# ZhengyiLuo/PULSE

Hardware: NVIDIA H100
Metric: env-steps/sec at 16384 humanoid envs, 1/2/4/8 H100; obs-kernel HBM GB/s (higher is better)
Workload: dtype bf16 GEMM operands, fp32 accumulate / master weights / observations

## Files before the change

### pulse_b200/csrc/gemm_kernel.inc

```
#if PULSE_GEMM_GROUPED
#define PULSE_GEMM_FIRST(member) grp.p[0].member
#define PULSE_GEMM_W wl
#define PULSE_GEMM_SELECT(w)                                                                                         \
  int pi = 0;                                                                                                        \
  while (pi + 1 < grp.count && (w) >= grp.p[pi].item_end) ++pi;                                                      \
  const GemmProblem& P = grp.p[pi];                                                                                  \
  const int wl = (w) - (pi == 0 ? 0 : grp.p[pi - 1].item_end);                                                       \
  const CUtensorMap& map_a = P.map_a;                                                                                \
  const CUtensorMap& map_b = P.map_b;                                                                                \
  const CUtensorMap& map_c = P.map_c;                                                                                \
  const int use_tma_red = P.use_tma_red;                                                                             \
  const pulse_gemm_epilogue_t& ep = P.ep;                                                                            \
  const int M = P.M, N = P.N, K = P.K, kb_per_split = P.kb_per_split;                                                \
  const int tiles_n = (N + BN - 1) / BN, tiles_m = (M + BM - 1) / BM;                                                \
  const int tiles = tiles_m * tiles_n;                                                                               \
  const int num_kb_total = (K + BK - 1) / BK;                                                                        \
  (void)map_a; (void)map_b; (void)map_c; (void)use_tma_red; (void)ep; (void)M; (void)N; (void)tiles_n; (void)kb_per_split; (void)num_kb_total;
#else
#define PULSE_GEMM_FIRST(member) member
#define PULSE_GEMM_W w
#define PULSE_GEMM_SELECT(w)
#endif

#if PULSE_GEMM_GROUPED
template <bool A_MN, bool B_MN, int MODE>
__global__ void __launch_bounds__(kThreads, 1) gemm_bf16_grouped_kernel(const __grid_constant__ GemmGroup grp) {
#else
template <bool A_MN, bool B_MN, int MODE>
__global__ void __launch_bounds__(kThreads, 1) gemm_bf16_kernel(const __grid_constant__ CUtensorMap map_a,
                                                                const __grid_constant__ CUtensorMap map_b,
                                                                const __grid_constant__ CUtensorMap map_c,
                                                                const pulse_gemm_epilogue_t ep, int M, int N, int K,
                                                                int kb_per_split, int splits, int use_tma_red) {
#endif
  constexpr bool kFwd = MODE == kModeGeneric || MODE == kModeFwd;
  constexpr bool kDgrad = MODE == kModeGeneric || MODE == kModeDgrad || MODE == kModeDgradVec;
  constexpr bool kGateVec = MODE == kModeGeneric || MODE == kModeDgradVec;
  constexpr bool kAccum = MODE == kModeGeneric || MODE == kModeWgrad;
  constexpr bool kBf16Out = MODE != kModeWgrad;
  extern __shared__ unsigned char gsm_raw[];
  GemmSmem& sm = *reinterpret_cast<GemmSmem*>((reinterpret_cast<uintptr_t>(gsm_raw) + 1023) & ~static_cast<uintptr_t>(1023));
  const int warp = threadIdx.x >> 5, lane = threadIdx.x & 31;
  const int work0 = static_cast<int>(blockIdx.x);
  const int work_stride = static_cast<int>(gridDim.x);
#if PULSE_GEMM_GROUPED
  const int total = grp.total_items;
#else
  const int tiles_n = (N + BN - 1) / BN, tiles_m = (M + BM - 1) / BM;
  const int tiles = tiles_m * tiles_n;
  const int total = tiles * splits;
  const int num_kb_total = (K + BK - 1) / BK;
#endif
  if (threadIdx.x == 0) PULSE_TRACE(0);

  if (threadIdx.x == 0) {
#pragma unroll
    for (int s = 0; s < kStages; ++s) {
      g_mbar_init(&sm.full[s], 1);
      g_mbar_init(&sm.empty[s], kConsumerWarps);
    }
    asm volatile("fence.mbarrier_init.release.cluster;\n" ::: "memory");
    asm volatile("prefetch.tensormap [%0];\n" ::"l"(&PULSE_GEMM_FIRST(map_a)) : "memory");
    asm volatile("prefetch.tensormap [%0];\n" ::"l"(&PULSE_GEMM_FIRST(map_b)) : "memory");
  }
  __syncthreads();
  if (threadIdx.x == 0) PULSE_TRACE(1);
  asm volatile("griddepcontrol.launch_dependents;\n" ::: "memory");

  if (warp < 4) {
    if (warp == 0 && lane == 0) {
      asm volatile("griddepcontrol.wait;\n" ::: "memory");
      PULSE_TRACE(2);
// ... 9 lines not shown
          g_mbar_wait(&sm.empty[s], ((it / kStages) & 1) ^ 1);
          g_mbar_expect_tx(&sm.full[s], kStageBytesA + kStageBytesB);
          const int kk = (kb0 + kb) * BK;
          if (A_MN) {
            tma_load_2d(sm.a[s], &map_a, m0, kk, &sm.full[s]);
            tma_load_2d(sm.a[s] + 8192, &map_a, m0 + 64, kk, &sm.full[s]);
          } else {
            tma_load_2d(sm.a[s], &map_a, kk, m0, &sm.full[s]);
          }
          if (B_MN) {
            tma_load_2d(sm.b[s], &map_b, n0, kk, &sm.full[s]);
            tma_load_2d(sm.b[s] + 8192, &map_b, n0 + 64, kk, &sm.full[s]);
          } else {
            tma_load_2d(sm.b[s], &map_b, kk, n0, &sm.full[s]);
          }
        }
      }
    }
  } else {
    const int wg = (warp >> 2) - 1;
    const int ew = warp - 4;
    const int quarter = wg * 2 + (warp & 1);
    const int chalf = (warp >> 1) & 1;
    float* red_stage = sm.red[ew];
    float* acc_s = sm.acc[wg];
    asm volatile("griddepcontrol.wait;\n" ::: "memory");
    int it = 0, lw = 0;
    for (int w = work0; w < total; w += work_stride, ++lw) {
      PULSE_GEMM_SELECT(w)
      const int split = PULSE_GEMM_W / tiles, t = PULSE_GEMM_W - split * tiles;
      const int m0 = (t / tiles_n) * BM, n0 = (t % tiles_n) * BN;
      const int kb0 = split * kb_per_split;
      const int num_kb = min(kb_per_split, num_kb_total - kb0);
      const int row = m0 + quarter * 32 + lane;
      const bool row_ok = row < M;
      const bool gate_fast = (MODE == kModeGeneric || MODE == kModeDgrad) && ep.gate != nullptr && ep.gate_mask == nullptr && ep.gate_mode == PULSE_ACT_RELU && (ep.ldg & 7) == 0 && n0 + chalf * kCols + kCols <= N;
      unsigned gmask[kChunks] = {};
      const bool gate_bits = kDgrad && ep.gate_mask != nullptr;
      if (gate_bits && row_ok) {
#pragma unroll
        for (int cc = 0; cc < kChunks; ++cc) {
          const int col = n0 + (chalf * kChunks + cc) * 32;
          if (col < N) gmask[cc] = __ldg(ep.gate_mask + static_cast<long long>(col >> 5) * ep.ld_gmask + row);
        }
      }
      if (gate_fast && row_ok) {
        const uint4* g = reinterpret_cast<const uint4*>(reinterpret_cast<const __nv_bfloat16*>(ep.gate) + static_cast<long long>(row) * ep.ldg +
                                                        n0 + chalf * kCols);
        uint4 u[kChunks * 4];
#pragma unroll
        for (int i = 0; i < kChunks * 4; ++i) u[i] = __ldg(g + i);
#pragma unroll
        for (int i = 0; i < kChunks * 4; ++i) {
          const unsigned wds[4] = {u[i].x, u[i].y, u[i].z, u[i].w};
#pragma unroll
          for (int q = 0; q < 4; ++q) {
            const unsigned pos = (((wds[q] & 0x7fff7fffu) + 0x7fff7fffu) & ~wds[q]) & 0x80008000u;
            gmask[i >> 2] |= (pos >> 15) << ((i & 3) * 4 + q);
          }
        }
      }
      const bool gate_vec = kGateVec && ep.gate != nullptr && !gate_fast && !gate_bits && (ep.ldg & 7) == 0;
      uint4 gq[4] = {};
      auto gate_fetch = [&](int cc) {
        const int c0 = n0 + cc * 32;
        if (gate_vec && row_ok && c0 + 32 <= N) {
          const uint4* g = reinterpret_cast<const uint4*>(reinterpret_cast<const __nv_bfloat16*>(ep.gate) + static_cast<long long>(row) * ep.ldg + c0);
#pragma unroll
          for (int q = 0; q < 4; ++q) gq[q] = __ldg(g + q);
        }
      };
      gate_fetch(chalf * kChunks);
      float bias_l[kChunks] = {};
      const bool fwd_fast = MODE == kModeFwd && ep.out != nullptr && (ep.ldo & 7) == 0 && ep.out_f32 == nullptr && ep.out_t == nullptr &&
                            (ep.preact == nullptr || (ep.ldp & 7) == 0) && n0 + chalf * kCols + kCols <= N;
      float* bias_s = sm.bias[ew];
      if (fwd_fast && ep.bias != nullptr) {
        __syncwarp();
#pragma unroll
        for (int cc = 0; cc < kChunks; ++cc) bias_s[cc * 32 + lane] = __ldg(ep.bias + n0 + (chalf * kChunks + cc) * 32 + lane);
        __syncwarp();
      } else if (kFwd && ep.bias != nullptr) {
#pragma unroll
        for (int cc = 0; cc < kChunks; ++cc) {
          const int col = n0 + (chalf * kChunks + cc) * 32 + lane;
          if (col < N) bias_l[cc] = __ldg(ep.bias + col);
        }
      }

      float d[64];
#pragma unroll
      for (int i = 0; i < 64; ++i) d[i] = 0.0f;
      acc_fence(d);
      int prev_s = -1;
      for (int kb = 0; kb < num_kb; ++kb, ++it) {
        const int s = it % kStages;
        g_mbar_wait(&sm.full[s], (it / kStages) & 1);
        if (it == 0 && ew == 0 && lane == 0) PULSE_TRACE(3);
        wgmma_fence();
        const unsigned a_addr = s_u32(sm.a[s]) + static_cast<unsigned>(wg) * 8192u, b_addr = s_u32(sm.b[s]);
#pragma unroll
        for (int k = 0; k < BK / MMA_K; ++k) {
          const unsigned long long da = A_MN ? gmma_desc(a_addr + k * 2048, 8192) : gmma_desc(a_addr + k * 32, 16);
          const unsigned long long db = B_MN ? gmma_desc(b_addr + k * 2048, 8192) : gmma_desc(b_addr + k * 32, 16);
          wgmma_m64n128<A_MN ? 1 : 0, B_MN ? 1 : 0>(d, da, db, (kb | k) != 0 ? 1u : 0u);
        }
        wgmma_commit();
        wgmma_wait<1>();
        if (prev_s >= 0 && lane == 0) g_mbar_arrive(&sm.empty[prev_s]);
        prev_s = s;
      }
      wgmma_wait<0>();
      acc_fence(d);
      if (lane == 0) g_mbar_arrive(&sm.empty[prev_s]);
      if (ew == 0 && lane == 0 && lw < 3) PULSE_TRACE(4 + lw);

      wg_sync(wg);
      {
        const int r0 = (warp & 3) * 16 + (lane >> 2);
#pragma unroll
        for (int j = 0; j < BN / 8; ++j) {
          const int col = 8 * j + 2 * (lane & 3);
#pragma unroll
          for (int h = 0; h < 2; ++h) {
            const int r = r0 + 8 * h;
            const int rb = r & 31;
            float* blk = acc_s + ((r >> 5) * 4 + (col >> 5)) * 1024;
            const int unit = ((col & 31) >> 2) ^ (rb & 7);
            *reinterpret_cast<float2*>(blk + rb * 32 + unit * 4 + (col & 3)) = make_float2(d[4 * j + 2 * h], d[4 * j + 2 * h + 1]);
          }
        }
      }
      if (MODE == kModeWgrad && use_tma_red) asm volatile("fence.proxy.async.shared::cta;\n" ::: "memory");
      wg_sync(wg);
      if (ew == 0 && lane == 0 && lw < 3) PULSE_TRACE(16 + 2 * lw);

      float* outf = ep.out_f32 != nullptr ? ep.out_f32 + static_cast<long long>(ep.accumulate ? 0 : split) * ep.split_stride : nullptr;
      float sq = 0.0f;
#pragma unroll 1
      for (int c = chalf * kChunks; c < chalf * kChunks + kChunks; ++c) {
        const int col0 = n0 + c * 32;
        const bool full = col0 + 32 <= N;
        float* blk = acc_s + ((quarter & 1) * 4 + c) * 1024;
        if (MODE == kModeWgrad && use_tma_red) {
          if (lane == 0) {
            asm volatile("cp.reduce.async.bulk.tensor.2d.global.shared::cta.add.tile.bulk_group [%0, {%2, %3}], [%1];\n" ::"l"(&map_c),
                         "r"(s_u32(blk)), "r"(col0), "r"(m0 + quarter * 32)
                         : "memory");
            asm volatile("cp.async.bulk.commit_group;\n" ::: "memory");
          }
          continue;
        }
        float v[32];
        {
          const float4* b4 = reinterpret_cast<const float4*>(blk) + lane * 8;
#pragma unroll
          for (int u = 0; u < 8; ++u) {
            const float4 x = b4[u ^ (lane & 7)];
            v[4 * u] = x.x; v[4 * u + 1] = x.y; v[4 * u + 2] = x.z; v[4 * u + 3] = x.w;
          }
        }
        if (MODE != kModeWgrad && ep.alpha != 1.0f) {
#pragma unroll
          for (int i = 0; i < 32; ++i) v[i] *= ep.alpha;
        }
        if (fwd_fast) {
          if (ep.bias != nullptr) {
            const float4* b4 = reinterpret_cast<const float4*>(bias_s + (c % kChunks) * 32);
#pragma unroll
            for (int i = 0; i < 32; i += 4) {
              const float4 b = b4[i >> 2];
              v[i] += b.x; v[i + 1] += b.y; v[i + 2] += b.z; v[i + 3] += b.w;
            }
          }
          if (ep.relu_mask != nullptr) {
            unsigned word = 0u;
#pragma unroll
            for (int i = 0; i < 32; ++i) word |= (v[i] > 0.0f ? 1u : 0u) << i;
            if (row_ok) ep.relu_mask[static_cast<long long>(col0 >> 5) * ep.ld_rmask + row] = word;
          }
          uint4* st = reinterpret_cast<uint4*>(red_stage);
          const int sw = (lane >> 1) & 3;
#pragma unroll
          for (int q = 0; q < 4; ++q) {
            const int i = 8 * q;
            __nv_bfloat162 h0 = __floats2bfloat162_rn(v[i], v[i + 1]), h1 = __floats2bfloat162_rn(v[i + 2], v[i + 3]);
            __nv_bfloat162 h2 = __floats2bfloat162_rn(v[i + 4], v[i + 5]), h3 = __floats2bfloat162_rn(v[i + 6], v[i + 7]);
            uint4 u;
            u.x = *reinterpret_cast<unsigned*>(&h0);
            u.y = *reinterpret_cast<unsigned*>(&h1);
            u.z = *reinterpret_cast<unsigned*>(&h2);
            u.w = *reinterpret_cast<unsigned*>(&h3);
            st[lane * 4 + (q ^ sw)] = u;
          }
          __syncwarp();
          const long long coff = col0 + (lane & 3) * 8;
          const __nv_bfloat162 zero2 = __float2bfloat162_rn(0.0f);
#pragma unroll
          for (int it2 = 0; it2 < 4; ++it2) {
            const int rr = it2 * 8 + (lane >> 2);
            uint4 u = st[rr * 4 + ((lane & 3) ^ ((rr >> 1) & 3))];
            __nv_bfloat162* h = reinterpret_cast<__nv_bfloat162*>(&u);
            const long long grow = m0 + quarter * 32 + rr;
            if (grow < M) {
              if (ep.preact != nullptr) *reinterpret_cast<uint4*>(reinterpret_cast<__nv_bfloat16*>(ep.preact) + grow * ep.ldp + coff) = u;
              if (ep.act == PULSE_ACT_RELU) {
#pragma unroll
                for (int q = 0; q < 4; ++q) h[q] = __hmax2(h[q], zero2);
              } else if (ep.act == PULSE_ACT_SILU) {
#pragma unroll
                for (int q = 0; q < 4; ++q) h[q] = silu_bf16x2(h[q]);
              }
              *reinterpret_cast<uint4*>(reinterpret_cast<__nv_bfloat16*>(ep.out) + grow * ep.ldo + coff) = u;
            }
          }
          __syncwarp();
          continue;
        }
        if (kFwd && ep.bias != nullptr) {
          float bl = bias_l[0];
#pragma unroll
          for (int cc = 1; cc < kChunks; ++cc) bl = (c % kChunks) == cc ? bias_l[cc] : bl;
#pragma unroll
          for (int i = 0; i < 32; ++i) v[i] += __shfl_sync(0xffffffffu, bl, i);
        }
        if (kFwd && ep.preact != nullptr) {
          if (full && (ep.ldp & 7) == 0) {
            store_block_bf16(reinterpret_cast<uint4*>(red_stage), v,
                             reinterpret_cast<__nv_bfloat16*>(ep.preact) + static_cast<long long>(m0 + quarter * 32) * ep.ldp + col0, ep.ldp,
                             M - (m0 + quarter * 32), lane);
          } else if (row_ok) {
            __nv_bfloat16* p = reinterpret_cast<__nv_bfloat16*>(ep.preact) + static_cast<long long>(row) * ep.ldp + col0;
#pragma unroll
            for (int i = 0; i < 32; ++i)
              if (col0 + i < N) p[i] = __float2bfloat16(v[i]);
          }
        }
        if (kFwd && ep.relu_mask != nullptr && row_ok) {
          unsigned word = 0u;
#pragma unroll
          for (int i = 0; i < 32; ++i) word |= ((col0 + i < N && v[i] > 0.0f) ? 1u : 0u) << i;
          if (col0 < N) ep.relu_mask[static_cast<long long>(col0 >> 5) * ep.ld_rmask + row] = word;
        }
        if (kFwd && ep.act != PULSE_ACT_NONE) {
#pragma unroll
          for (int i = 0; i < 32; ++i) v[i] = act_apply(v[i], ep.act);
        }
        if (gate_bits) {
          unsigned mk = gmask[0];
#pragma unroll
// ... 64 lines not shown
            }
            __syncwarp();
          }
        } else if (outf != nullptr && row_ok) {
          float* p = outf + static_cast<long long>(row) * ep.ldf + col0;
          if (full && (ep.ldf & 3) == 0 && (reinterpret_cast<uintptr_t>(outf) & 15u) == 0) {
#pragma unroll
            for (int i = 0; i < 32; i += 4) *reinterpret_cast<float4*>(p + i) = make_float4(v[i], v[i + 1], v[i + 2], v[i + 3]);
          } else {
#pragma unroll
            for (int i = 0; i < 32; ++i)
              if (col0 + i < N) p[i] = v[i];
          }
        }
        if (kBf16Out && ep.out != nullptr) {
          if (full && (ep.ldo & 7) == 0) {
            store_block_bf16(reinterpret_cast<uint4*>(red_stage), v,
                             reinterpret_cast<__nv_bfloat16*>(ep.out) + static_cast<long long>(m0 + quarter * 32) * ep.ldo + col0, ep.ldo,
                             M - (m0 + quarter * 32), lane);
          } else if (row_ok) {
            __nv_bfloat16* p = reinterpret_cast<__nv_bfloat16*>(ep.out) + static_cast<long long>(row) * ep.ldo + col0;
#pragma unroll
            for (int i = 0; i < 32; ++i)
              if (col0 + i < N) p[i] = __float2bfloat16(v[i]);
          }
        }
        if (kFwd && ep.out_t != nullptr && row_ok) {
#pragma unroll
          for (int i = 0; i < 32; ++i)
            if (col0 + i < N)
              reinterpret_cast<__nv_bfloat16*>(ep.out_t)[static_cast<long long>(col0 + i) * ep.ldot + row] = __float2bfloat16(v[i]);
        }
      }
      if (MODE == kModeWgrad && use_tma_red) {
        if (lane == 0) asm volatile("cp.async.bulk.wait_group.read 0;\n" ::: "memory");
        __syncwarp();
      }
      if (kDgrad && ep.sumsq != nullptr) {
#pragma unroll
        for (int o = 16; o > 0; o >>= 1) sq += __shfl_xor_sync(0xffffffffu, sq, o);
        if (lane == 0) atomicAdd(ep.sumsq, static_cast<double>(sq));
      }
      if (ew == 0 && lane == 0 && lw < 3) PULSE_TRACE(17 + 2 * lw);
    }
  }
  if (MODE == kModeWgrad && warp >= 4 && lane == 0) asm volatile("cp.async.bulk.wait_group 0;\n" ::: "memory");
  if (threadIdx.x == 0) PULSE_TRACE(10);
}


#undef PULSE_GEMM_FIRST
#undef PULSE_GEMM_W
#undef PULSE_GEMM_SELECT
```

### pulse_b200/csrc/gemm_wgmma.cu

```cuda
#include <cuda.h>
#include <stdlib.h>
#include <string.h>
#include <cuda_bf16.h>

#include "pulse_common.cuh"

namespace pulse {
namespace {

#ifndef PULSE_GEMM_VARIANT
#define PULSE_GEMM_VARIANT 0
#endif
constexpr int BM = 128, BN = 128, BK = 64, MMA_K = 16;
constexpr int kConsumerWarps = 8;
constexpr int kThreads = 128 + 32 * kConsumerWarps;
constexpr int kCols = 64;
constexpr int kChunks = kCols / 32;
constexpr int kStages = 4;
constexpr unsigned kStageBytesA = BM * BK * 2;
constexpr unsigned kStageBytesB = BN * BK * 2;

struct __align__(1024) GemmSmem {
  unsigned char a[kStages][kStageBytesA];
  unsigned char b[kStages][kStageBytesB];
  float acc[2][64 * BN];
  float red[kConsumerWarps][16 * 33];
  float bias[kConsumerWarps][kCols];
  unsigned long long full[kStages];
  unsigned long long empty[kStages];
};

__device__ __forceinline__ unsigned s_u32(const void* p) { return static_cast<unsigned>(__cvta_generic_to_shared(p)); }
__device__ __forceinline__ void g_mbar_init(unsigned long long* bar, unsigned count) {
  asm volatile("mbarrier.init.shared::cta.b64 [%0], %1;\n" ::"r"(s_u32(bar)), "r"(count));
}
__device__ __forceinline__ void g_mbar_expect_tx(unsigned long long* bar, unsigned bytes) {
  asm volatile("mbarrier.arrive.expect_tx.shared::cta.b64 _, [%0], %1;\n" ::"r"(s_u32(bar)), "r"(bytes) : "memory");
}
__device__ __forceinline__ void g_mbar_arrive(unsigned long long* bar) {
  asm volatile("mbarrier.arrive.shared::cta.b64 _, [%0];\n" ::"r"(s_u32(bar)) : "memory");
}
__device__ __forceinline__ bool g_mbar_try(unsigned long long* bar, unsigned parity) {
  unsigned ok;
  asm volatile(
      "{\n\t.reg .pred p;\n\t"
      "mbarrier.try_wait.parity.shared::cta.b64 p, [%1], %2;\n\t"
      "selp.u32 %0, 1, 0, p;\n\t}\n"
      : "=r"(ok)
      : "r"(s_u32(bar)), "r"(parity)
      : "memory");
  return ok != 0;
}
__device__ __forceinline__ void g_mbar_wait(unsigned long long* bar, unsigned parity) {
  for (int spin = 0; spin < (1 << 26); ++spin)
    if (g_mbar_try(bar, parity)) return;
  __trap();
}
__device__ __forceinline__ void tma_load_2d(void* smem_dst, const CUtensorMap* map, int c0, int c1, unsigned long long* bar) {
  asm volatile("cp.async.bulk.tensor.2d.shared::cluster.global.mbarrier::complete_tx::bytes [%0], [%1, {%3, %4}], [%2];\n" ::"r"(
                   s_u32(smem_dst)),
               "l"(map), "r"(s_u32(bar)), "r"(c0), "r"(c1)
               : "memory");
}
__device__ __forceinline__ void wg_sync(int wg) { asm volatile("bar.sync %0, 128;\n" ::"r"(1 + wg) : "memory"); }

__device__ __forceinline__ unsigned long long gmma_desc(unsigned smem_addr, unsigned lbo) {
  unsigned long long d = 0;
  d |= static_cast<unsigned long long>((smem_addr >> 4) & 0x3fffu);
  d |= static_cast<unsigned long long>((lbo >> 4) & 0x3fffu) << 16;
  d |= static_cast<unsigned long long>(1024u >> 4) << 32;
  d |= static_cast<unsigned long long>(1u) << 62;
  return d;
}
__device__ __forceinline__ void wgmma_fence() { asm volatile("wgmma.fence.sync.aligned;\n" ::: "memory"); }
__device__ __forceinline__ void wgmma_commit() { asm volatile("wgmma.commit_group.sync.aligned;\n" ::: "memory"); }
template <int N>
__device__ __forceinline__ void wgmma_wait() { asm volatile("wgmma.wait_group.sync.aligned %0;\n" ::"n"(N) : "memory"); }
__device__ __forceinline__ void acc_fence(float (&d)[64]) {
#pragma unroll
  for (int i = 0; i < 64; ++i) asm volatile("" : "+f"(d[i])::"memory");
}
template <int TA, int TB>
__device__ __forceinline__ void wgmma_m64n128(float (&d)[64], unsigned long long da, unsigned long long db, unsigned accumulate) {
  asm volatile(
      "{\n\t.reg .pred p;\n\t"
      "setp.ne.b32 p, %66, 0;\n\t"
      "wgmma.mma_async.sync.aligned.m64n128k16.f32.bf16.bf16 "
      "{%0, %1, %2, %3, %4, %5, %6, %7, %8, %9, %10, %11, %12, %13, %14, %15, %16, %17, %18, %19, %20, %21, %22, %23, %24, %25, %26, "
      "%27, %28, %29, %30, %31, %32, %33, %34, %35, %36, %37, %38, %39, %40, %41, %42, %43, %44, %45, %46, %47, %48, %49, %50, %51, "
      "%52, %53, %54, %55, %56, %57, %58, %59, %60, %61, %62, %63}, "
      "%64, %65, p, 1, 1, %67, %68;\n\t}\n"
      : "+f"(d[0]), "+f"(d[1]), "+f"(d[2]), "+f"(d[3]), "+f"(d[4]), "+f"(d[5]), "+f"(d[6]), "+f"(d[7]),
        "+f"(d[8]), "+f"(d[9]), "+f"(d[10]), "+f"(d[11]), "+f"(d[12]), "+f"(d[13]), "+f"(d[14]), "+f"(d[15]),
        "+f"(d[16]), "+f"(d[17]), "+f"(d[18]), "+f"(d[19]), "+f"(d[20]), "+f"(d[21]), "+f"(d[22]), "+f"(d[23]),
        "+f"(d[24]), "+f"(d[25]), "+f"(d[26]), "+f"(d[27]), "+f"(d[28]), "+f"(d[29]), "+f"(d[30]), "+f"(d[31]),
// ... 34 lines not shown
    u.w = *reinterpret_cast<unsigned*>(&h3);
    st[lane * 4 + (q ^ sw)] = u;
  }
  __syncwarp();
  __nv_bfloat16* obase = base + (lane & 3) * 8;
#pragma unroll
  for (int it = 0; it < 4; ++it) {
    const int rr = it * 8 + (lane >> 2);
    const uint4 val = st[rr * 4 + ((lane & 3) ^ ((rr >> 1) & 3))];
    if (rr < rows_valid) *reinterpret_cast<uint4*>(obase + static_cast<long long>(rr) * ld) = val;
  }
  __syncwarp();
}

#if PULSE_GEMM_VARIANT == 3
__device__ long long g_gemm_trace[32];
#define PULSE_TRACE(slot)                                          \
  do {                                                             \
    if (blockIdx.x == 0) g_gemm_trace[slot] = clock64();           \
  } while (0)
#else
#define PULSE_TRACE(slot) \
  do {                    \
  } while (0)
#endif

__device__ __forceinline__ __nv_bfloat162 silu_bf16x2(__nv_bfloat162 z) {
  float2 f = __bfloat1622float2(z);
  f.x = __fdividef(f.x, 1.0f + __expf(-f.x));
  f.y = __fdividef(f.y, 1.0f + __expf(-f.y));
  return __floats2bfloat162_rn(f.x, f.y);
}

enum : int { kModeGeneric = 0, kModeFwd = 1, kModeDgrad = 2, kModeWgrad = 3, kModeDgradVec = 4 };

constexpr int kMaxGroup = 4;
struct GemmProblem {
  CUtensorMap map_a, map_b, map_c;
  pulse_gemm_epilogue_t ep;
  int M, N, K, kb_per_split;
  int item_end;
  int use_tma_red;
  int pad[2];
};
struct GemmGroup {
  GemmProblem p[kMaxGroup];
  int count, total_items;
};

#define PULSE_GEMM_GROUPED 0
#include "gemm_kernel.inc"
#undef PULSE_GEMM_GROUPED
#define PULSE_GEMM_GROUPED 1
#include "gemm_kernel.inc"
#undef PULSE_GEMM_GROUPED

typedef CUresult (*EncodeTiledFn)(CUtensorMap*, CUtensorMapDataType, cuuint32_t, void*, const cuuint64_t*, const cuuint64_t*,
                                  const cuuint32_t*, const cuuint32_t*, CUtensorMapInterleave, CUtensorMapSwizzle,
                                  CUtensorMapL2promotion, CUtensorMapFloatOOBfill);
EncodeTiledFn get_encode_fn() {
  static EncodeTiledFn fn = nullptr;
  if (fn == nullptr) {
    void* p = nullptr;
    cudaDriverEntryPointQueryResult q;
    if (cudaGetDriverEntryPoint("cuTensorMapEncodeTiled", &p, cudaEnableDefault, &q) == cudaSuccess && q == cudaDriverEntryPointSuccess)
      fn = reinterpret_cast<EncodeTiledFn>(p);
  }
  return fn;
}

bool make_map(CUtensorMap* map, const void* base, long long rows, long long cols, long long ld, unsigned box_rows) {
  EncodeTiledFn fn = get_encode_fn();
  if (fn == nullptr) return false;
  cuuint64_t dims[2] = {static_cast<cuuint64_t>(cols), static_cast<cuuint64_t>(rows)};
  cuuint64_t strides[1] = {static_cast<cuuint64_t>(ld) * 2};
  cuuint32_t box[2] = {BK, box_rows};
  cuuint32_t estr[2] = {1, 1};
  return fn(map, CU_TENSOR_MAP_DATA_TYPE_BFLOAT16, 2, const_cast<void*>(base), dims, strides, box, estr, CU_TENSOR_MAP_INTERLEAVE_NONE,
            CU_TENSOR_MAP_SWIZZLE_128B, CU_TENSOR_MAP_L2_PROMOTION_L2_256B, CU_TENSOR_MAP_FLOAT_OOB_FILL_NONE) == CUDA_SUCCESS;
}

bool make_map_c(CUtensorMap* map, const float* base, long long rows, long long cols, long long ld) {
  EncodeTiledFn fn = get_encode_fn();
  if (fn == nullptr) return false;
  cuuint64_t dims[2] = {static_cast<cuuint64_t>(cols), static_cast<cuuint64_t>(rows)};
  cuuint64_t strides[1] = {static_cast<cuuint64_t>(ld) * 4};
  cuuint32_t box[2] = {32, 32};
  cuuint32_t estr[2] = {1, 1};
  return fn(map, CU_TENSOR_MAP_DATA_TYPE_FLOAT32, 2, const_cast<float*>(base), dims, strides, box, estr, CU_TENSOR_MAP_INTERLEAVE_NONE,
            CU_TENSOR_MAP_SWIZZLE_128B, CU_TENSOR_MAP_L2_PROMOTION_NONE, CU_TENSOR_MAP_FLOAT_OOB_FILL_NONE) == CUDA_SUCCESS;
}
bool tma_reduce_ok(const pulse_gemm_epilogue_t& ep) {
  return ep.out_f32 != nullptr && ep.accumulate && (ep.ldf % 4) == 0 && (reinterpret_cast<uintptr_t>(ep.out_f32) % 16) == 0;
}

constexpr size_t kSmemBytes = sizeof(GemmSmem) + 1024;

int gemm_num_sms(bool honour_limit) {
  static int num_sms = 0, limited = 0;
  if (num_sms == 0) {
    int dev = 0;
    if (cudaGetDevice(&dev) != cudaSuccess || cudaDeviceGetAttribute(&num_sms, cudaDevAttrMultiProcessorCount, dev) != cudaSuccess) return 0;
    limited = num_sms;
    const char* e = getenv("PULSE_GEMM_SMS");
    if (e != nullptr && atoi(e) >= 1 && atoi(e) < num_sms) limited = atoi(e);
  }
  return honour_limit ? limited : num_sms;
}

template <bool A_MN, bool B_MN, int MODE>
int launch_gemm(const CUtensorMap& map_a, const CUtensorMap& map_b, const pulse_gemm_epilogue_t& ep, int m, int n, int k, int splits,
                int kb_per_split, cudaStream_t stream) {
  static bool attr_set = false;
  CUtensorMap map_c;
  memset(&map_c, 0, sizeof(map_c));
  int use_tma_red = 0;
  if (MODE == kModeWgrad && tma_reduce_ok(ep)) {
    if (!make_map_c(&map_c, ep.out_f32, m, n, ep.ldf)) {
      set_error("pulse_gemm_bf16: cuTensorMapEncodeTiled failed for the fp32 output");
      return PULSE_ERR_CUDA;
    }
    use_tma_red = 1;
  }
  if (!attr_set) {
    PULSE_CUDA_OK(cudaFuncSetAttribute(gemm_bf16_kernel<A_MN, B_MN, MODE>, cudaFuncAttributeMaxDynamicSharedMemorySize, (int)kSmemBytes));
    attr_set = true;
  }
  const int num_sms = gemm_num_sms(true);
  PULSE_REQUIRE(num_sms > 0, "pulse_gemm_bf16: cannot query the device's SM count");
  const long long total = static_cast<long long>((n + BN - 1) / BN) * ((m + BM - 1) / BM) * splits;
  const unsigned grid = static_cast<unsigned>(total < num_sms ? total : num_sms);
  static int use_pdl = -1;
  if (use_pdl < 0) {
    const char* e = getenv("PULSE_GEMM_PDL");
    use_pdl = (e != nullptr && e[0] == '0') ? 0 : 1;
  }
  cudaLaunchConfig_t cfg = {};
  cfg.gridDim = dim3(grid, 1, 1);
  cfg.blockDim = dim3(kThreads, 1, 1);
  cfg.dynamicSmemBytes = kSmemBytes;
  cfg.stream = stream;
  cudaLaunchAttribute attr[1];
  int na = 0;
  if (use_pdl) {
    attr[na].id = cudaLaunchAttributeProgrammaticStreamSerialization;
    attr[na].val.programmaticStreamSerializationAllowed = 1;
    ++na;
  }
  cfg.attrs = attr;
  cfg.numAttrs = na;
  PULSE_CUDA_OK(cudaLaunchKernelEx(&cfg, gemm_bf16_kernel<A_MN, B_MN, MODE>, map_a, map_b, map_c, ep, m, n, k, kb_per_split, splits, use_tma_red));
  PULSE_LAUNCH_OK("gemm_bf16_kernel");
  return PULSE_OK;
}

template <bool A_MN, bool B_MN, int MODE>
int launch_gemm_grouped(const GemmGroup& grp, cudaStream_t stream) {
  static bool attr_set = false;
  if (!attr_set) {
    PULSE_CUDA_OK(cudaFuncSetAttribute(gemm_bf16_grouped_kernel<A_MN, B_MN, MODE>, cudaFuncAttributeMaxDynamicSharedMemorySize, (int)kSmemBytes));
    attr_set = true;
  }
  const int num_sms = gemm_num_sms(false);
  PULSE_REQUIRE(num_sms > 0, "pulse_gemm_bf16_grouped: cannot query the device's SM count");
  const unsigned grid = static_cast<unsigned>(grp.total_items < num_sms ? grp.total_items : num_sms);
  cudaLaunchConfig_t cfg = {};
  cfg.gridDim = dim3(grid, 1, 1);
  cfg.blockDim = dim3(kThreads, 1, 1);
  cfg.dynamicSmemBytes = kSmemBytes;
  cfg.stream = stream;
  cudaLaunchAttribute attr[1];
  attr[0].id = cudaLaunchAttributeProgrammaticStreamSerialization;
  attr[0].val.programmaticStreamSerializationAllowed = 1;
  cfg.attrs = attr;
  cfg.numAttrs = 1;
  PULSE_CUDA_OK(cudaLaunchKernelEx(&cfg, gemm_bf16_grouped_kernel<A_MN, B_MN, MODE>, grp));
  PULSE_LAUNCH_OK("gemm_bf16_grouped_kernel");
  return PULSE_OK;
}

int epilogue_mode(const pulse_gemm_epilogue_t* ep) {
  const bool want_fwd = ep->bias || ep->act != PULSE_ACT_NONE || ep->preact || ep->out_t || ep->relu_mask;
  const bool want_dgrad = ep->gate || ep->colsum || ep->sumsq || ep->gate_mask;
  const bool want_accum = ep->accumulate != 0;
// ... 81 lines not shown
  for (int i = 0; i < count; ++i) {
    const pulse_gemm_problem_t& q = problems[i];
    PULSE_REQUIRE(q.a && q.b, "pulse_gemm_bf16_grouped: null operand in problem %d", i);
    PULSE_REQUIRE(q.m > 0 && q.n > 0 && q.k > 0 && q.m < (1ll << 31) && q.n < (1ll << 31) && q.k < (1ll << 31), "pulse_gemm_bf16_grouped: bad shape in problem %d", i);
    PULSE_REQUIRE(q.lda >= (a_mn ? q.m : q.k) && q.ldb >= (b_mn ? q.n : q.k) && (q.lda % 8) == 0 && (q.ldb % 8) == 0,
                  "pulse_gemm_bf16_grouped: leading dimensions of problem %d must cover the contiguous extent and be multiples of 8", i);
    PULSE_REQUIRE(aligned16(q.a) && aligned16(q.b), "pulse_gemm_bf16_grouped: operands of problem %d must be 16-byte aligned", i);
    PULSE_REQUIRE(q.ep.out || q.ep.out_t || q.ep.out_f32, "pulse_gemm_bf16_grouped: problem %d has no output", i);
    PULSE_REQUIRE(q.split_k >= 1, "pulse_gemm_bf16_grouped: split_k must be >= 1");
    PULSE_REQUIRE(q.split_k == 1 || (q.ep.out_f32 && q.ep.accumulate && !q.ep.out && !q.ep.out_t && !q.ep.bias && q.ep.act == PULSE_ACT_NONE && !q.ep.gate &&
                                     !q.ep.preact && !q.ep.colsum),
                  "pulse_gemm_bf16_grouped: split-K only with fp32 atomic accumulation");
    const int mq = epilogue_mode(&q.ep);
    PULSE_REQUIRE(mode < 0 || mq == mode, "pulse_gemm_bf16_grouped: problem %d needs a different epilogue specialisation than problem 0", i);
    mode = mq;
  }
  PULSE_REQUIRE(mode == kModeFwd || mode == kModeDgrad || mode == kModeWgrad, "pulse_gemm_bf16_grouped: forward, ReLU-dgrad and wgrad groups only");
  PULSE_REQUIRE((mode == kModeFwd && !a_mn && !b_mn) || (mode == kModeDgrad && !a_mn && b_mn) || (mode == kModeWgrad && a_mn && b_mn),
                "pulse_gemm_bf16_grouped: operand majors do not match the group kind (fwd K/K, dgrad K/MN, wgrad MN/MN)");
  GemmGroup grp;
  memset(&grp, 0, sizeof(grp));
  grp.count = count;
  long long items = 0;
  for (int i = 0; i < count; ++i) {
    const pulse_gemm_problem_t& q = problems[i];
    GemmProblem& g = grp.p[i];
    const bool ok_a = a_mn ? make_map(&g.map_a, q.a, q.k, q.m, q.lda, 64) : make_map(&g.map_a, q.a, q.m, q.k, q.lda, BM);
    const bool ok_b = b_mn ? make_map(&g.map_b, q.b, q.k, q.n, q.ldb, 64) : make_map(&g.map_b, q.b, q.n, q.k, q.ldb, BN);
    if (!ok_a || !ok_b) {
      set_error("pulse_gemm_bf16_grouped: cuTensorMapEncodeTiled failed for problem %d", i);
      return PULSE_ERR_CUDA;
    }
    g.ep = q.ep;
    g.use_tma_red = 0;
    if (mode == kModeWgrad && tma_reduce_ok(q.ep)) {
      if (!make_map_c(&g.map_c, q.ep.out_f32, q.m, q.n, q.ep.ldf)) {
        set_error("pulse_gemm_bf16_grouped: cuTensorMapEncodeTiled failed for the fp32 output of problem %d", i);
        return PULSE_ERR_CUDA;
      }
      g.use_tma_red = 1;
    }
    g.M = static_cast<int>(q.m);
    g.N = static_cast<int>(q.n);
    g.K = static_cast<int>(q.k);
    const int num_kb = static_cast<int>((q.k + BK - 1) / BK);
    const int splits = pulse_gemm_num_splits(q.k, q.split_k);
    g.kb_per_split = (num_kb + splits - 1) / splits;
    items += static_cast<long long>((q.n + BN - 1) / BN) * ((q.m + BM - 1) / BM) * splits;
    PULSE_REQUIRE(items < (1ll << 30), "pulse_gemm_bf16_grouped: too many work items");
    g.item_end = static_cast<int>(items);
  }
  grp.total_items = static_cast<int>(items);
  cudaStream_t st = static_cast<cudaStream_t>(stream);
  if (mode == kModeFwd) return launch_gemm_grouped<false, false, kModeFwd>(grp, st);
  if (mode == kModeDgrad) return launch_gemm_grouped<false, true, kModeDgrad>(grp, st);
  return launch_gemm_grouped<true, true, kModeWgrad>(grp, st);
}
```

Baseline: 1.787 million.

## Stage GEMM forward/dgrad epilogue in registers with stmatrix and TMA bf16 stores

Forward and ReLU-dgrad GEMMs whose outputs meet the TMA alignment rules now apply alpha, bias, ReLU-mask bit packing and gate masking directly on the WGMMA accumulator registers. The result goes to shared memory through stmatrix and is written to global memory with TMA bulk tensor stores, for both the output and the pre-activation. This skips the fp32 accumulator round trip through shared memory and the per-warp transpose and vector store path. The cost is extra tensor maps per problem, waits on outstanding bulk stores before the staging buffer is reused, and a more complex mask-shuffle path that is only correct when the layout assumptions hold.

```diff
diff --git a/pulse_b200/csrc/gemm_kernel.inc b/pulse_b200/csrc/gemm_kernel.inc
--- a/pulse_b200/csrc/gemm_kernel.inc
+++ b/pulse_b200/csrc/gemm_kernel.inc
@@ -9,13 +9,14 @@
   const CUtensorMap& map_a = P.map_a;                                                                                \
   const CUtensorMap& map_b = P.map_b;                                                                                \
   const CUtensorMap& map_c = P.map_c;                                                                                \
-  const int use_tma_red = P.use_tma_red;                                                                             \
+  const CUtensorMap& map_p = P.map_p;                                                                                \
+  const int tma_out = P.tma_out;                                                                                     \
   const pulse_gemm_epilogue_t& ep = P.ep;                                                                            \
   const int M = P.M, N = P.N, K = P.K, kb_per_split = P.kb_per_split;                                                \
   const int tiles_n = (N + BN - 1) / BN, tiles_m = (M + BM - 1) / BM;                                                \
   const int tiles = tiles_m * tiles_n;                                                                               \
   const int num_kb_total = (K + BK - 1) / BK;                                                                        \
-  (void)map_a; (void)map_b; (void)map_c; (void)use_tma_red; (void)ep; (void)M; (void)N; (void)tiles_n; (void)kb_per_split; (void)num_kb_total;
+  (void)map_a; (void)map_b; (void)map_c; (void)map_p; (void)tma_out; (void)ep; (void)M; (void)N; (void)tiles_n; (void)kb_per_split; (void)num_kb_total;
 #else
 #define PULSE_GEMM_FIRST(member) member
 #define PULSE_GEMM_W w
@@ -30,14 +31,16 @@
 __global__ void __launch_bounds__(kThreads, 1) gemm_bf16_kernel(const __grid_constant__ CUtensorMap map_a,
                                                                 const __grid_constant__ CUtensorMap map_b,
                                                                 const __grid_constant__ CUtensorMap map_c,
+                                                                const __grid_constant__ CUtensorMap map_p,
                                                                 const pulse_gemm_epilogue_t ep, int M, int N, int K,
-                                                                int kb_per_split, int splits, int use_tma_red) {
+                                                                int kb_per_split, int splits, int tma_out) {
 #endif
   constexpr bool kFwd = MODE == kModeGeneric || MODE == kModeFwd;
   constexpr bool kDgrad = MODE == kModeGeneric || MODE == kModeDgrad || MODE == kModeDgradVec;
   constexpr bool kGateVec = MODE == kModeGeneric || MODE == kModeDgradVec;
   constexpr bool kAccum = MODE == kModeGeneric || MODE == kModeWgrad;
   constexpr bool kBf16Out = MODE != kModeWgrad;
+  constexpr bool kRegEpi = MODE == kModeFwd || MODE == kModeDgrad;
   extern __shared__ unsigned char gsm_raw[];
   GemmSmem& sm = *reinterpret_cast<GemmSmem*>((reinterpret_cast<uintptr_t>(gsm_raw) + 1023) & ~static_cast<uintptr_t>(1023));
   const int warp = threadIdx.x >> 5, lane = threadIdx.x & 31;
@@ -113,12 +116,23 @@
       const int m0 = (t / tiles_n) * BM, n0 = (t % tiles_n) * BN;
       const int kb0 = split * kb_per_split;
       const int num_kb = min(kb_per_split, num_kb_total - kb0);
+      const bool reg_epi = kRegEpi && tma_out;
+      const int r0 = (warp & 3) * 16 + (lane >> 2);
       const int row = m0 + quarter * 32 + lane;
       const bool row_ok = row < M;
       const bool gate_fast = (MODE == kModeGeneric || MODE == kModeDgrad) && ep.gate != nullptr && ep.gate_mask == nullptr && ep.gate_mode == PULSE_ACT_RELU && (ep.ldg & 7) == 0 && n0 + chalf * kCols + kCols <= N;
-      unsigned gmask[kChunks] = {};
+      unsigned gmask[8] = {};
       const bool gate_bits = kDgrad && ep.gate_mask != nullptr;
-      if (gate_bits && row_ok) {
+      if (gate_bits && reg_epi) {
+#pragma unroll
+        for (int c = 0; c < 4; ++c) {
+#pragma unroll
+          for (int h = 0; h < 2; ++h) {
+            const int r = m0 + wg * 64 + r0 + 8 * h;
+            if (r < M && n0 + c * 32 < N) gmask[2 * c + h] = __ldg(ep.gate_mask + static_cast<long long>((n0 >> 5) + c) * ep.ld_gmask + r);
+          }
+        }
+      } else if (gate_bits && row_ok) {
 #pragma unroll
         for (int cc = 0; cc < kChunks; ++cc) {
           const int col = n0 + (chalf * kChunks + cc) * 32;
@@ -153,14 +167,9 @@
       };
       gate_fetch(chalf * kChunks);
       float bias_l[kChunks] = {};
-      const bool fwd_fast = MODE == kModeFwd && ep.out != nullptr && (ep.ldo & 7) == 0 && ep.out_f32 == nullptr && ep.out_t == nullptr &&
-                            (ep.preact == nullptr || (ep.ldp & 7) == 0) && n0 + chalf * kCols + kCols <= N;
-      float* bias_s = sm.bias[ew];
-      if (fwd_fast && ep.bias != nullptr) {
-        __syncwarp();
-#pragma unroll
-        for (int cc = 0; cc < kChunks; ++cc) bias_s[cc * 32 + lane] = __ldg(ep.bias + n0 + (chalf * kChunks + cc) * 32 + lane);
-        __syncwarp();
+      if (reg_epi && kFwd && ep.bias != nullptr) {
+        const int t = (warp & 3) * 32 + lane;
+        sm.bias[wg][t] = n0 + t < N ? __ldg(ep.bias + n0 + t) : 0.0f;
       } else if (kFwd && ep.bias != nullptr) {
 #pragma unroll
         for (int cc = 0; cc < kChunks; ++cc) {
@@ -196,9 +205,100 @@
       if (lane == 0) g_mbar_arrive(&sm.empty[prev_s]);
       if (ew == 0 && lane == 0 && lw < 3) PULSE_TRACE(4 + lw);
 
+      if (kRegEpi && (warp & 3) == 0 && lane == 0) asm volatile("cp.async.bulk.wait_group.read 0;\n" ::: "memory");
       wg_sync(wg);
+      float sq = 0.0f;
+
+      if (reg_epi) {
+        const int q = lane & 3;
+        if (ep.alpha != 1.0f) {
+#pragma unroll
+          for (int i = 0; i < 64; ++i) d[i] *= ep.alpha;
+        }
+        if (kFwd && ep.bias != nullptr) {
+          const float* bs = sm.bias[wg] + 2 * q;
+#pragma unroll
+          for (int j = 0; j < BN / 8; ++j) {
+            const float2 b = *reinterpret_cast<const float2*>(bs + 8 * j);
+            d[4 * j] += b.x; d[4 * j + 1] += b.y; d[4 * j + 2] += b.x; d[4 * j + 3] += b.y;
+          }
+        }
+        if (kFwd && ep.relu_mask != nullptr) {
+          unsigned wd[4][2];
+#pragma unroll
+          for (int c = 0; c < 4; ++c) {
+#pragma unroll
+            for (int h = 0; h < 2; ++h) {
+              unsigned b = 0u;
+#pragma unroll
+              for (int jj = 0; jj < 4; ++jj)
+#pragma unroll
+                for (int e = 0; e < 2; ++e) b |= (d[4 * (4 * c + jj) + 2 * h + e] > 0.0f ? 1u : 0u) << (8 * jj + e);
+              wd[c][h] = b << (2 * q);
+            }
+          }
+          const bool up2 = (q & 2) != 0, up1 = (q & 1) != 0;
+          unsigned wf[2];
+#pragma unroll
+          for (int h = 0; h < 2; ++h) {
+            unsigned w2[2];
+#pragma unroll
+            for (int k = 0; k < 2; ++k) w2[k] = (up2 ? wd[k + 2][h] : wd[k][h]) | __shfl_xor_sync(0xffffffffu, up2 ? wd[k][h] : wd[k + 2][h], 2);
+            wf[h] = (up1 ? w2[1] : w2[0]) | __shfl_xor_sync(0xffffffffu, up1 ? w2[0] : w2[1], 1);
+          }
+          const int col0 = n0 + 32 * q;
+          if (col0 < N) {
+            const unsigned valid = N - col0 >= 32 ? 0xffffffffu : (1u << (N - col0)) - 1u;
+#pragma unroll
+            for (int h = 0; h < 2; ++h) {
+              const int r = m0 + wg * 64 + r0 + 8 * h;
+              if (r < M) ep.relu_mask[static_cast<long long>(col0 >> 5) * ep.ld_rmask + r] = wf[h] & valid;
+            }
+          }
+        }
+        if (gate_bits) {
+#pragma unroll
+          for (int c = 0; c < 4; ++c) {
+#pragma unroll
+            for (int h = 0; h < 2; ++h) {
+              const unsigned mk = gmask[2 * c + h] >> (2 * q);
+#pragma unroll
+              for (int jj = 0; jj < 4; ++jj)
+#pragma unroll
+                for (int e = 0; e < 2; ++e) {
+                  float& x = d[4 * (4 * c + jj) + 2 * h + e];
+                  x = ((mk >> (8 * jj + e)) & 1u) ? x : 0.0f;
+                }
+            }
+          }
+        }
+        if (kDgrad && ep.sumsq != nullptr) {
+#pragma unroll
+          for (int i = 0; i < 64; ++i) sq = fmaf(d[i], d[i], sq);
+        }
+        const unsigned stage = s_u32(acc_s);
+        const bool pre = kFwd && ep.preact != nullptr;
+        if (!kFwd || ep.act == PULSE_ACT_NONE) stage_tile_bf16<PULSE_ACT_NONE>(d, stage, pre, n0, N);
+        else if (ep.act == PULSE_ACT_RELU) stage_tile_bf16<PULSE_ACT_RELU>(d, stage, pre, n0, N);
+        else stage_tile_bf16<PULSE_ACT_SILU>(d, stage, pre, n0, N);
+        asm volatile("fence.proxy.async.shared::cta;\n" ::: "memory");
+        wg_sync(wg);
+        if (ew == 0 && lane == 0 && lw < 3) PULSE_TRACE(16 + 2 * lw);
+        if ((warp & 3) == 0 && lane == 0 && m0 + wg * 64 < M) {
+#pragma unroll
+          for (int b = 0; b < 2; ++b) {
+            if (n0 + 64 * b >= N) continue;
+            tma_store_2d(&map_c, stage + b * 8192, n0 + 64 * b, m0 + wg * 64);
+            if (pre) tma_store_2d(&map_p, stage + 16384 + b * 8192, n0 + 64 * b, m0 + wg * 64);
+          }
+          asm volatile("cp.async.bulk.commit_group;\n" ::: "memory");
+        }
+        if (kDgrad && ep.sumsq != nullptr) add_sumsq(ep.sumsq, sq);
+        if (ew == 0 && lane == 0 && lw < 3) PULSE_TRACE(17 + 2 * lw);
+        continue;
+      }
+
       {
-        const int r0 = (warp & 3) * 16 + (lane >> 2);
 #pragma unroll
         for (int j = 0; j < BN / 8; ++j) {
           const int col = 8 * j + 2 * (lane & 3);
@@ -212,18 +312,17 @@
           }
         }
       }
-      if (MODE == kModeWgrad && use_tma_red) asm volatile("fence.proxy.async.shared::cta;\n" ::: "memory");
+      if (MODE == kModeWgrad && tma_out) asm volatile("fence.proxy.async.shared::cta;\n" ::: "memory");
       wg_sync(wg);
       if (ew == 0 && lane == 0 && lw < 3) PULSE_TRACE(16 + 2 * lw);
 
       float* outf = ep.out_f32 != nullptr ? ep.out_f32 + static_cast<long long>(ep.accumulate ? 0 : split) * ep.split_stride : nullptr;
-      float sq = 0.0f;
 #pragma unroll 1
       for (int c = chalf * kChunks; c < chalf * kChunks + kChunks; ++c) {
         const int col0 = n0 + c * 32;
         const bool full = col0 + 32 <= N;
         float* blk = acc_s + ((quarter & 1) * 4 + c) * 1024;
-        if (MODE == kModeWgrad && use_tma_red) {
+        if (MODE == kModeWgrad && tma_out) {
           if (lane == 0) {
             asm volatile("cp.reduce.async.bulk.tensor.2d.global.shared::cta.add.tile.bulk_group [%0, {%2, %3}], [%1];\n" ::"l"(&map_c),
                          "r"(s_u32(blk)), "r"(col0), "r"(m0 + quarter * 32)
@@ -244,59 +343,6 @@
         if (MODE != kModeWgrad && ep.alpha != 1.0f) {
 #pragma unroll
           for (int i = 0; i < 32; ++i) v[i] *= ep.alpha;
-        }
-        if (fwd_fast) {
-          if (ep.bias != nullptr) {
-            const float4* b4 = reinterpret_cast<const float4*>(bias_s + (c % kChunks) * 32);
-#pragma unroll
-            for (int i = 0; i < 32; i += 4) {
-              const float4 b = b4[i >> 2];
-              v[i] += b.x; v[i + 1] += b.y; v[i + 2] += b.z; v[i + 3] += b.w;
-            }
-          }
-          if (ep.relu_mask != nullptr) {
-            unsigned word = 0u;
-#pragma unroll
-            for (int i = 0; i < 32; ++i) word |= (v[i] > 0.0f ? 1u : 0u) << i;
-            if (row_ok) ep.relu_mask[static_cast<long long>(col0 >> 5) * ep.ld_rmask + row] = word;
-          }
-          uint4* st = reinterpret_cast<uint4*>(red_stage);
-          const int sw = (lane >> 1) & 3;
-#pragma unroll
-          for (int q = 0; q < 4; ++q) {
-            const int i = 8 * q;
-            __nv_bfloat162 h0 = __floats2bfloat162_rn(v[i], v[i + 1]), h1 = __floats2bfloat162_rn(v[i + 2], v[i + 3]);
-            __nv_bfloat162 h2 = __floats2bfloat162_rn(v[i + 4], v[i + 5]), h3 = __floats2bfloat162_rn(v[i + 6], v[i + 7]);
-            uint4 u;
-            u.x = *reinterpret_cast<unsigned*>(&h0);
-            u.y = *reinterpret_cast<unsigned*>(&h1);
-            u.z = *reinterpret_cast<unsigned*>(&h2);
-            u.w = *reinterpret_cast<unsigned*>(&h3);
-            st[lane * 4 + (q ^ sw)] = u;
-          }
-          __syncwarp();
-          const long long coff = col0 + (lane & 3) * 8;
-          const __nv_bfloat162 zero2 = __float2bfloat162_rn(0.0f);
-#pragma unroll
-          for (int it2 = 0; it2 < 4; ++it2) {
-            const int rr = it2 * 8 + (lane >> 2);
-            uint4 u = st[rr * 4 + ((lane & 3) ^ ((rr >> 1) & 3))];
-            __nv_bfloat162* h = reinterpret_cast<__nv_bfloat162*>(&u);
-            const long long grow = m0 + quarter * 32 + rr;
-            if (grow < M) {
-              if (ep.preact != nullptr) *reinterpret_cast<uint4*>(reinterpret_cast<__nv_bfloat16*>(ep.preact) + grow * ep.ldp + coff) = u;
-              if (ep.act == PULSE_ACT_RELU) {
-#pragma unroll
-                for (int q = 0; q < 4; ++q) h[q] = __hmax2(h[q], zero2);
-              } else if (ep.act == PULSE_ACT_SILU) {
-#pragma unroll
-                for (int q = 0; q < 4; ++q) h[q] = silu_bf16x2(h[q]);
-              }
-              *reinterpret_cast<uint4*>(reinterpret_cast<__nv_bfloat16*>(ep.out) + grow * ep.ldo + coff) = u;
-            }
-          }
-          __syncwarp();
-          continue;
         }
         if (kFwd && ep.bias != nullptr) {
           float bl = bias_l[0];
@@ -427,19 +473,15 @@
               reinterpret_cast<__nv_bfloat16*>(ep.out_t)[static_cast<long long>(col0 + i) * ep.ldot + row] = __float2bfloat16(v[i]);
         }
       }
-      if (MODE == kModeWgrad && use_tma_red) {
+      if (MODE == kModeWgrad && tma_out) {
         if (lane == 0) asm volatile("cp.async.bulk.wait_group.read 0;\n" ::: "memory");
         __syncwarp();
       }
-      if (kDgrad && ep.sumsq != nullptr) {
-#pragma unroll
-        for (int o = 16; o > 0; o >>= 1) sq += __shfl_xor_sync(0xffffffffu, sq, o);
-        if (lane == 0) atomicAdd(ep.sumsq, static_cast<double>(sq));
-      }
+      if (kDgrad && ep.sumsq != nullptr) add_sumsq(ep.sumsq, sq);
       if (ew == 0 && lane == 0 && lw < 3) PULSE_TRACE(17 + 2 * lw);
     }
   }
-  if (MODE == kModeWgrad && warp >= 4 && lane == 0) asm volatile("cp.async.bulk.wait_group 0;\n" ::: "memory");
+  if ((MODE == kModeWgrad || kRegEpi) && warp >= 4 && lane == 0) asm volatile("cp.async.bulk.wait_group 0;\n" ::: "memory");
   if (threadIdx.x == 0) PULSE_TRACE(10);
 }
 
diff --git a/pulse_b200/csrc/gemm_wgmma.cu b/pulse_b200/csrc/gemm_wgmma.cu
--- a/pulse_b200/csrc/gemm_wgmma.cu
+++ b/pulse_b200/csrc/gemm_wgmma.cu
@@ -25,7 +25,7 @@
   unsigned char b[kStages][kStageBytesB];
   float acc[2][64 * BN];
   float red[kConsumerWarps][16 * 33];
-  float bias[kConsumerWarps][kCols];
+  float bias[2][BN];
   unsigned long long full[kStages];
   unsigned long long empty[kStages];
 };
@@ -61,6 +61,20 @@
                    s_u32(smem_dst)),
                "l"(map), "r"(s_u32(bar)), "r"(c0), "r"(c1)
                : "memory");
+}
+__device__ __forceinline__ void tma_store_2d(const CUtensorMap* map, unsigned smem_src, int c0, int c1) {
+  asm volatile("cp.async.bulk.tensor.2d.global.shared::cta.bulk_group [%0, {%2, %3}], [%1];\n" ::"l"(map), "r"(smem_src), "r"(c0), "r"(c1)
+               : "memory");
+}
+__device__ __forceinline__ void stmatrix_x4(unsigned addr, const unsigned (&r)[4]) {
+  asm volatile("stmatrix.sync.aligned.m8n8.x4.shared.b16 [%0], {%1, %2, %3, %4};\n" ::"r"(addr), "r"(r[0]), "r"(r[1]), "r"(r[2]), "r"(r[3])
+               : "memory");
+}
+__device__ __forceinline__ unsigned bf16x2_bits(__nv_bfloat162 h) { return *reinterpret_cast<unsigned*>(&h); }
+__device__ __forceinline__ void add_sumsq(double* sumsq, float sq) {
+#pragma unroll
+  for (int o = 16; o > 0; o >>= 1) sq += __shfl_xor_sync(0xffffffffu, sq, o);
+  if ((threadIdx.x & 31) == 0) atomicAdd(sumsq, static_cast<double>(sq));
 }
 __device__ __forceinline__ void wg_sync(int wg) { asm volatile("bar.sync %0, 128;\n" ::"r"(1 + wg) : "memory"); }
 
@@ -161,15 +175,40 @@
   return __floats2bfloat162_rn(f.x, f.y);
 }
 
+template <int ACT>
+__device__ __forceinline__ void stage_tile_bf16(const float (&d)[64], unsigned stage, bool pre, int n0, int N) {
+  const int lane = threadIdx.x & 31, warp = threadIdx.x >> 5;
+  const unsigned srow = stage + ((warp & 3) * 16 + ((lane >> 3) & 1) * 8 + (lane & 7)) * 128;
+  const int sj = lane >> 4;
+  const __nv_bfloat162 zero2 = __float2bfloat162_rn(0.0f);
+#pragma unroll
+  for (int j = 0; j < BN / 8; j += 2) {
+    const bool full_half = n0 + 64 * (j >> 3) + 64 <= N;
+    unsigned o[4], p[4];
+#pragma unroll
+    for (int k = 0; k < 4; ++k) {
+      const int i = 4 * (j + (k >> 1)) + 2 * (k & 1);
+      __nv_bfloat162 h = __floats2bfloat162_rn(d[i], d[i + 1]);
+      p[k] = bf16x2_bits(h);
+      if (ACT == PULSE_ACT_RELU) h = __hmax2(h, zero2);
+      if (ACT == PULSE_ACT_SILU) h = full_half ? silu_bf16x2(h) : __floats2bfloat162_rn(act_apply(d[i], ACT), act_apply(d[i + 1], ACT));
+      o[k] = bf16x2_bits(h);
+    }
+    const unsigned addr = srow + (j >> 3) * 8192 + ((((j & 7) + sj) ^ (lane & 7)) << 4);
+    stmatrix_x4(addr, o);
+    if (pre) stmatrix_x4(addr + 16384, p);
+  }
+}
+
 enum : int { kModeGeneric = 0, kModeFwd = 1, kModeDgrad = 2, kModeWgrad = 3, kModeDgradVec = 4 };
 
 constexpr int kMaxGroup = 4;
 struct GemmProblem {
-  CUtensorMap map_a, map_b, map_c;
+  CUtensorMap map_a, map_b, map_c, map_p;
   pulse_gemm_epilogue_t ep;
   int M, N, K, kb_per_split;
   int item_end;
-  int use_tma_red;
+  int tma_out;
   int pad[2];
 };
 struct GemmGroup {
@@ -222,6 +261,31 @@
 bool tma_reduce_ok(const pulse_gemm_epilogue_t& ep) {
   return ep.out_f32 != nullptr && ep.accumulate && (ep.ldf % 4) == 0 && (reinterpret_cast<uintptr_t>(ep.out_f32) % 16) == 0;
 }
+bool tma_rows_ok(const void* base, long long ld) { return (ld % 8) == 0 && (reinterpret_cast<uintptr_t>(base) % 16) == 0; }
+
+int epilogue_maps(int mode, const pulse_gemm_epilogue_t& ep, long long m, long long n, CUtensorMap* map_c, CUtensorMap* map_p, int* tma_out) {
+  memset(map_c, 0, sizeof(*map_c));
+  memset(map_p, 0, sizeof(*map_p));
+  *tma_out = 0;
+  if (mode == kModeWgrad) {
+    if (!tma_reduce_ok(ep)) return PULSE_OK;
+    if (!make_map_c(map_c, ep.out_f32, m, n, ep.ldf)) {
+      set_error("pulse_gemm_bf16: cuTensorMapEncodeTiled failed for the fp32 output");
+      return PULSE_ERR_CUDA;
+    }
+    *tma_out = 1;
+    return PULSE_OK;
+  }
+  if ((mode != kModeFwd && mode != kModeDgrad) || (n % 8) != 0 || ep.out == nullptr || ep.out_f32 != nullptr || ep.out_t != nullptr || ep.gate != nullptr ||
+      ep.colsum != nullptr || !tma_rows_ok(ep.out, ep.ldo) || (ep.preact != nullptr && !tma_rows_ok(ep.preact, ep.ldp)))
+    return PULSE_OK;
+  if (!make_map(map_c, ep.out, m, n, ep.ldo, 64) || (ep.preact != nullptr && !make_map(map_p, ep.preact, m, n, ep.ldp, 64))) {
+    set_error("pulse_gemm_bf16: cuTensorMapEncodeTiled failed for the bf16 output");
+    return PULSE_ERR_CUDA;
+  }
+  *tma_out = 1;
+  return PULSE_OK;
+}
 
 constexpr size_t kSmemBytes = sizeof(GemmSmem) + 1024;
 
@@ -241,16 +305,10 @@
 int launch_gemm(const CUtensorMap& map_a, const CUtensorMap& map_b, const pulse_gemm_epilogue_t& ep, int m, int n, int k, int splits,
                 int kb_per_split, cudaStream_t stream) {
   static bool attr_set = false;
-  CUtensorMap map_c;
-  memset(&map_c, 0, sizeof(map_c));
-  int use_tma_red = 0;
-  if (MODE == kModeWgrad && tma_reduce_ok(ep)) {
-    if (!make_map_c(&map_c, ep.out_f32, m, n, ep.ldf)) {
-      set_error("pulse_gemm_bf16: cuTensorMapEncodeTiled failed for the fp32 output");
-      return PULSE_ERR_CUDA;
-    }
-    use_tma_red = 1;
-  }
+  CUtensorMap map_c, map_p;
+  int tma_out = 0;
+  const int rc = epilogue_maps(MODE, ep, m, n, &map_c, &map_p, &tma_out);
+  if (rc != PULSE_OK) return rc;
   if (!attr_set) {
     PULSE_CUDA_OK(cudaFuncSetAttribute(gemm_bf16_kernel<A_MN, B_MN, MODE>, cudaFuncAttributeMaxDynamicSharedMemorySize, (int)kSmemBytes));
     attr_set = true;
@@ -278,7 +336,7 @@
   }
   cfg.attrs = attr;
   cfg.numAttrs = na;
-  PULSE_CUDA_OK(cudaLaunchKernelEx(&cfg, gemm_bf16_kernel<A_MN, B_MN, MODE>, map_a, map_b, map_c, ep, m, n, k, kb_per_split, splits, use_tma_red));
+  PULSE_CUDA_OK(cudaLaunchKernelEx(&cfg, gemm_bf16_kernel<A_MN, B_MN, MODE>, map_a, map_b, map_c, map_p, ep, m, n, k, kb_per_split, splits, tma_out));
   PULSE_LAUNCH_OK("gemm_bf16_kernel");
   return PULSE_OK;
 }
@@ -426,14 +484,8 @@
       return PULSE_ERR_CUDA;
     }
     g.ep = q.ep;
-    g.use_tma_red = 0;
-    if (mode == kModeWgrad && tma_reduce_ok(q.ep)) {
-      if (!make_map_c(&g.map_c, q.ep.out_f32, q.m, q.n, q.ep.ldf)) {
-        set_error("pulse_gemm_bf16_grouped: cuTensorMapEncodeTiled failed for the fp32 output of problem %d", i);
-        return PULSE_ERR_CUDA;
-      }
-      g.use_tma_red = 1;
-    }
+    const int rc = epilogue_maps(mode, q.ep, q.m, q.n, &g.map_c, &g.map_p, &g.tma_out);
+    if (rc != PULSE_OK) return rc;
     g.M = static_cast<int>(q.m);
     g.N = static_cast<int>(q.n);
     g.K = static_cast<int>(q.k);
```

New measurement: 1.875 million (median of 6 runs). 4.9% higher.
